# JamesKane/DecodingUsTools

Measured on NVIDIA B200. Metric: aligned Gbases/s CallableLoci pileup, higher is better.
Workload: dtype u8/u32 integer

## Files before the change

decodingustools_b200/csrc/callable_loci_b200.cu:

```cuda
#include "../../include/callable_loci_b200.h"
#include "clb_kernels.cuh"
#include "clb_fast.cuh"

#include <dlfcn.h>

#include <algorithm>
#include <cstdarg>
#include <cstdio>
#include <cstdlib>
#include <cstring>
#include <string>
#include <vector>

using namespace clb;

namespace {

struct DevBuf {
    void *p = nullptr;
    size_t cap = 0;
};

struct EvPair { cudaEvent_t a, b; };

// ... 13 lines not shown

    bool in_contig = false, finished = false;
    int32_t tid = 0;
    std::string name;
    uint32_t contig_len = 0, largest = 0, region_start = 0, region_end = 0;
    uint32_t n_windows = 0, windows_done = 0;
    uint32_t stride = 0, n_bins = 0;
    uint32_t dh_next = 0, dh_n = 0;
    uint32_t dh_fetched = 0;
    bool long_mode = false, span_on_device = false;
    uint64_t n_reads = 0, n_cigar = 0, n_qual = 0;
    long long last_pos = -1;

    DevBuf pos, flag, mapq, cigar_off, cigar, qual_off, qual, read_end, cigar_ckpt;
    DevBuf nmask, ref_ascii;
    DevBuf stats_padded, counters, rec, win_tab, win_rec, win_out, deep_list, intervals, misc;
    DevBuf gen_list, blk_tot, dhist;
    DevBuf dbg_raw, dbg_qc, dbg_low, dbg_state, timing;
    uint32_t rec_cap = 0;
    bool dbg = false;

    clb_interval *h_intervals = nullptr;
    size_t h_intervals_cap = 0;
    std::vector<unsigned long long> h_counters;
    std::vector<uint32_t> h_bins;
    uint32_t *h_misc = nullptr;
    uint64_t h2d_bytes = 0, d2h_bytes = 0;
    uint32_t launches = 0;
    uint64_t n_intervals = 0;
};

enum { M_CURSOR = 0, M_ERR = 1, M_NTOTAL = 2, M_DEEP = 3, M_GEN_COUNT = 4, M_GEN_TAKEN = 5, M_RESET_WORDS = 6, M_MAXSPAN = 7, M_MAXQLEN = 8, M_WORDS = 9 };

namespace {

int fail(clb_ctx *c, int code, const char *fmt, ...) {
    char buf[512];
    va_list ap; va_start(ap, fmt); vsnprintf(buf, sizeof buf, fmt, ap); va_end(ap);
    if (c) c->err = buf;
    return code;
}

#define CU(call)                                                                                              \
    do {                                                                                                      \
        cudaError_t e_ = (call);                                                                              \
        if (e_ != cudaSuccess) return fail(ctx, CLB_E_CUDA, "%s failed: %s (%s:%d)", #call, cudaGetErrorString(e_), __FILE__, __LINE__); \
    } while (0)
// ... 33 lines not shown
KParams make_params(clb_ctx *c) {
    KParams P{};
    P.pos = (const int32_t *)c->pos.p; P.flag = (const uint16_t *)c->flag.p; P.mapq = (const uint8_t *)c->mapq.p;
    P.cigar_off = (const uint32_t *)c->cigar_off.p; P.cigar = (const uint32_t *)c->cigar.p;
    P.qual_off = (const uint64_t *)c->qual_off.p; P.qual = (const uint8_t *)c->qual.p; P.qual_bytes = c->qual.cap;
    P.read_end = c->long_mode ? (const uint32_t *)c->read_end.p : nullptr;
    P.cigar_ckpt = c->long_mode ? (const uint2 *)c->cigar_ckpt.p : nullptr;
    P.nmask = (const uint32_t *)c->nmask.p;
    P.region_start = c->region_start; P.region_end = c->region_end;
    P.min_depth = c->opt.min_depth; P.max_depth = c->opt.max_depth; P.min_depth_for_low_mapq = c->opt.min_depth_for_low_mapq;
    P.min_mapq = c->opt.min_mapping_quality; P.min_bq = c->opt.min_base_quality; P.max_low_mapq = c->opt.max_low_mapq;
    P.first_tab = c->d_first_tab;
    P.win_tables = c->d_first_tab + 65536;
    P.first_tab8 = (const uint8_t *)(c->d_first_tab + 65536) + WIN_TABLE_BYTES;
    P.win_rec = (const uint4 *)c->win_rec.p;
    P.stats = (unsigned long long *)c->stats_padded.p;
    P.bins = (unsigned long long *)c->counters.p + N_STATS;
    P.n_bins = c->n_bins; P.stride = c->stride;
    P.rec = (unsigned long long *)c->rec.p; P.rec_cap = c->rec_cap;
    P.rec_cursor = (uint32_t *)c->misc.p + M_CURSOR;
    P.win_tab = (uint2 *)c->win_tab.p;
    P.err = (uint32_t *)c->misc.p + M_ERR;
    P.deep_count = (uint32_t *)c->misc.p + M_DEEP; P.deep_list = (uint32_t *)c->deep_list.p;
    P.gen_list = (uint32_t *)c->gen_list.p;
    P.gen_count = (uint32_t *)c->misc.p + M_GEN_COUNT; P.gen_taken = (uint32_t *)c->misc.p + M_GEN_TAKEN;
    P.max_span = (const uint32_t *)c->misc.p + M_MAXSPAN;
    P.max_low_mapq_fraction = c->opt.max_low_mapq_fraction;
    P.timing = (long long *)c->timing.p;
    P.dhist = c->dh_n ? (unsigned long long *)c->dhist.p : nullptr; P.dh_n = c->dh_n;
    if (c->dbg) {
        P.dbg_raw = (uint32_t *)c->dbg_raw.p; P.dbg_qc = (uint32_t *)c->dbg_qc.p;
        P.dbg_low = (uint32_t *)c->dbg_low.p; P.dbg_state = (uint8_t *)c->dbg_state.p;
    }
    return P;
}

template <typename F>
void with_variant(bool bq_hi, bool dbg, bool hist, F &&f) {
    using T = std::true_type; using N = std::false_type;
    auto h = [&](auto b, auto d) { if (hist) f(b, d, T{}); else f(b, d, N{}); };
    if (bq_hi) { if (dbg) h(T{}, T{}); else h(T{}, N{}); }
    else { if (dbg) h(N{}, T{}); else h(N{}, N{}); }
}

int launch_windows(clb_ctx *ctx, uint32_t w0, uint32_t w1, EvPair *time_pileup = nullptr, EvPair *time_fast = nullptr) {
    if (w1 <= w0) return CLB_OK;
    const uint32_t n = w1 - w0;
    const bool all_general = ctx->force_general || ctx->long_mode;
    k_window_ranges<<<(unsigned)(((uint64_t)n * WR_LANES + 255) / 256), 256, 0, ctx->s_compute>>>(
        (const int32_t *)ctx->pos.p, (uint32_t)ctx->n_reads, ctx->region_start, ctx->region_end,
        (const uint32_t *)ctx->misc.p + M_MAXSPAN, w0, n, (const uint64_t *)ctx->qual_off.p, (const uint32_t *)ctx->cigar_off.p, ctx->stride,
        (uint4 *)ctx->win_rec.p, all_general ? 1u : 0u, (uint32_t *)ctx->gen_list.p, (uint32_t *)ctx->misc.p + M_GEN_COUNT,
        (const uint32_t *)ctx->misc.p + M_MAXQLEN);
    KParams P = make_params(ctx);
    P.win_first = w0;
    if (time_pileup) CU(cudaEventRecord(time_pileup->a, ctx->s_compute));
    const bool hi = ctx->opt.min_base_quality >= 128;
    if (!all_general) {
        if (time_fast) CU(cudaEventRecord(time_fast->a, ctx->s_compute));
        with_variant(hi, ctx->dbg, ctx->dh_n != 0, [&](auto h, auto d, auto x) {
            k_pileup_fast<decltype(h)::value, decltype(d)::value, decltype(x)::value><<<n, NT, F_SMEM, ctx->s_compute>>>(P);
        });
        if (time_fast) CU(cudaEventRecord(time_fast->b, ctx->s_compute));
        ctx->launches += 1;
    }
    const uint32_t g = (uint32_t)std::min<uint64_t>((uint64_t)ctx->n_sm * std::max(1, ctx->max_ctas_per_sm), all_general ? n : 0xffffffffu);
    with_variant(hi, ctx->dbg, ctx->dh_n != 0, [&](auto h, auto d, auto x) {
        k_pileup_general<decltype(h)::value, decltype(d)::value, decltype(x)::value><<<g, NT, SMEM_BYTES, ctx->s_compute>>>(P);
    });
    if (time_pileup) CU(cudaEventRecord(time_pileup->b, ctx->s_compute));
    ctx->launches += 2;
    CU(cudaGetLastError());
    return CLB_OK;
}

int reset_accumulators(clb_ctx *ctx) {
    CU(cudaMemsetAsync(ctx->stats_padded.p, 0, (size_t)N_STATS * STAT_STRIDE * 8, ctx->s_compute));
    CU(cudaMemsetAsync(ctx->counters.p, 0, n_counters(ctx) * 8, ctx->s_compute));
    if (ctx->dh_n) CU(cudaMemsetAsync(ctx->dhist.p, 0, (size_t)DH_SLOTS * 2 * ctx->dh_n * 8, ctx->s_compute));
    CU(cudaMemsetAsync((uint32_t *)ctx->misc.p + M_CURSOR, 0, M_RESET_WORDS * sizeof(uint32_t), ctx->s_compute));
    return CLB_OK;
}

int launch_compaction(clb_ctx *ctx) {
    if (ctx->n_windows == 0) return CLB_OK;
    {
        const KParams P = make_params(ctx);
        with_variant(ctx->opt.min_base_quality >= 128, ctx->dbg, ctx->dh_n != 0, [&](auto h, auto d, auto x) {
            k_pileup_classify_deep<decltype(h)::value, decltype(d)::value, decltype(x)::value><<<ctx->n_sm, NT, SMEM_BYTES_DEEP, ctx->s_compute>>>(P);
        });
        ctx->launches += 1;
    }
    const uint32_t n_blk = (ctx->n_windows + 1023) / 1024;
    k_scan_windows_local<<<n_blk, 1024, 0, ctx->s_compute>>>((const uint2 *)ctx->win_tab.p, ctx->n_windows, (uint32_t *)ctx->win_out.p,
                                                            (uint32_t *)ctx->blk_tot.p, (const uint32_t *)ctx->misc.p + M_ERR);
    k_scan_blocks<<<1, 1024, 0, ctx->s_compute>>>((uint32_t *)ctx->blk_tot.p, n_blk, (uint32_t *)ctx->misc.p + M_NTOTAL);
    const uint32_t warps_per_block = 8;
    k_gather_intervals<<<(ctx->n_windows + warps_per_block - 1) / warps_per_block, warps_per_block * 32, 0, ctx->s_compute>>>(
        (const unsigned long long *)ctx->rec.p, (const uint2 *)ctx->win_tab.p, (const uint32_t *)ctx->win_out.p,
        (const uint32_t *)ctx->blk_tot.p, ctx->n_windows, (IntervalOut *)ctx->intervals.p, (const uint32_t *)ctx->misc.p + M_ERR);
    k_fill_ends<<<std::max(1, ctx->n_sm * 4), 256, 0, ctx->s_compute>>>((IntervalOut *)ctx->intervals.p,
                                                                       (const uint32_t *)ctx->misc.p + M_NTOTAL, ctx->region_end,
                                                                       (const uint32_t *)ctx->misc.p + M_ERR);
    k_pack_stats<<<1, 32, 0, ctx->s_compute>>>((const unsigned long long *)ctx->stats_padded.p, (unsigned long long *)ctx->counters.p);
    ctx->launches += 5;
    if (ctx->dh_n) {
        const uint32_t n2 = 2 * ctx->dh_n;
        k_fold_depth_hist<<<(n2 + 255) / 256, 256, 0, ctx->s_compute>>>((const unsigned long long *)ctx->dhist.p, n2,
                                                                     (unsigned long long *)ctx->counters.p + N_STATS + 3 * (size_t)ctx->n_bins);
        ctx->launches += 1;
    }
    CU(cudaGetLastError());
    return CLB_OK;
}

int alloc_outputs(clb_ctx *ctx) {
    int rc;
    const size_t nw = std::max<size_t>(ctx->n_windows, 1);
    if ((rc = ensure(ctx, ctx->win_tab, nw * sizeof(uint2), false, ctx->s_compute))) return rc;
    if ((rc = ensure(ctx, ctx->win_rec, nw * 3 * sizeof(uint4), false, ctx->s_compute))) return rc;
    if ((rc = ensure(ctx, ctx->win_out, nw * 4, false, ctx->s_compute))) return rc;
    if ((rc = ensure(ctx, ctx->deep_list, nw * 4, false, ctx->s_compute))) return rc;
    if ((rc = ensure(ctx, ctx->gen_list, nw * 4, false, ctx->s_compute))) return rc;
    if ((rc = ensure(ctx, ctx->blk_tot, ((nw + 1023) / 1024 + 1) * 4, false, ctx->s_compute))) return rc;
    if ((rc = ensure(ctx, ctx->rec, (size_t)ctx->rec_cap * 8, false, ctx->s_compute))) return rc;
    if ((rc = ensure(ctx, ctx->intervals, (size_t)ctx->rec_cap * sizeof(IntervalOut), false, ctx->s_compute))) return rc;
    return CLB_OK;
}

int fetch_result(clb_ctx *ctx, clb_contig_result *out) {
    const size_t n_cnt = n_counters(ctx);
    ctx->dh_fetched = 0;
    ctx->h_counters.resize(n_cnt);
    CU(cudaMemcpyAsync(ctx->h_misc, ctx->misc.p, M_WORDS * 4, cudaMemcpyDeviceToHost, ctx->s_compute));
    CU(cudaMemcpyAsync(ctx->h_counters.data(), ctx->counters.p, n_cnt * 8, cudaMemcpyDeviceToHost, ctx->s_compute));
    CU(cudaStreamSynchronize(ctx->s_compute));
    const uint32_t e = ctx->h_misc[M_ERR];
    if (e & ERR_UNSORTED) return fail(ctx, CLB_E_INPUT, "read columns are not coordinate sorted (or pos < 0)");
    if (e & ERR_OFFSETS) return fail(ctx, CLB_E_INPUT, "cigar_off / qual_off are not monotone");
    if (e & ERR_QUAL_SPAN) return fail(ctx, CLB_E_UNSUPPORTED, "a window's candidate reads span more than 4 GiB of qualities");
    if (e & ERR_REC_OVERFLOW) return 1;
// ... 116 lines not shown
    cudaDeviceGetAttribute(&ctx->n_sm, cudaDevAttrMultiProcessorCount, device);
    if ((e = cudaMalloc((void **)&ctx->d_first_tab, 65536 * 4 + WIN_TABLE_BYTES + 256)) != cudaSuccess) { clb_destroy(ctx); return bail("cudaMalloc", e); }
    k_first_table<<<65536 / 256, 256, 0, ctx->s_compute>>>(ctx->d_first_tab, (uint8_t *)(ctx->d_first_tab + 65536) + WIN_TABLE_BYTES, opt->max_low_mapq_fraction);
    k_window_tables<<<1, 256, 0, ctx->s_compute>>>(ctx->d_first_tab + 65536, opt->max_low_mapq_fraction);
    if ((e = cudaHostAlloc((void **)&ctx->h_misc, M_WORDS * 4, cudaHostAllocDefault)) != cudaSuccess) { clb_destroy(ctx); return bail("cudaHostAlloc", e); }
    if ((e = cudaStreamSynchronize(ctx->s_compute)) != cudaSuccess) { clb_destroy(ctx); return bail("first-table kernel", e); }
    return ctx;
}

void clb_destroy(clb_ctx *ctx) {
    if (!ctx) return;
    cudaSetDevice(ctx->device);
    cudaDeviceSynchronize();
    for (DevBuf *b : {&ctx->pos, &ctx->flag, &ctx->mapq, &ctx->cigar_off, &ctx->cigar, &ctx->qual_off, &ctx->qual, &ctx->read_end, &ctx->cigar_ckpt,
                      &ctx->nmask, &ctx->ref_ascii, &ctx->stats_padded, &ctx->counters, &ctx->rec, &ctx->win_tab, &ctx->win_rec,
                      &ctx->win_out, &ctx->deep_list, &ctx->intervals, &ctx->misc, &ctx->gen_list, &ctx->blk_tot, &ctx->dhist, &ctx->dbg_raw, &ctx->dbg_qc, &ctx->dbg_low, &ctx->dbg_state, &ctx->timing})
        release(*b);
    if (ctx->d_first_tab) cudaFree(ctx->d_first_tab);
    if (ctx->h_intervals) cudaFreeHost(ctx->h_intervals);
    if (ctx->h_misc) cudaFreeHost(ctx->h_misc);
    for (auto &ep : ctx->ev_pool) { cudaEventDestroy(ep.a); cudaEventDestroy(ep.b); }
    for (auto &ep : ctx->ev_kernel) { cudaEventDestroy(ep.a); cudaEventDestroy(ep.b); }
    for (auto &ep : ctx->ev_h2d) { cudaEventDestroy(ep.a); cudaEventDestroy(ep.b); }
    for (auto &ep : ctx->ev_upload) { cudaEventDestroy(ep.a); cudaEventDestroy(ep.b); }
    if (ctx->ev_copy) cudaEventDestroy(ctx->ev_copy);
    if (ctx->s_own) cudaStreamDestroy(ctx->s_own);
    if (ctx->s_copy) cudaStreamDestroy(ctx->s_copy);
    delete ctx;
}

const char *clb_last_error(const clb_ctx *ctx) { return ctx ? ctx->err.c_str() : "null context"; }
// ... 344 lines not shown
```

decodingustools_b200/csrc/clb_fast.cuh:

```cuda
#pragma once
#include "clb_kernels.cuh"

namespace clb {

constexpr int F_CW = 520;
constexpr int F_WSTAGE = CLB_F_WSTAGE;
constexpr int F_XCAP = 96;
constexpr int F_MAXOPS = 64;
constexpr int F_LOOKBACK = 254;
constexpr int F_NFIRST = 256;
#ifndef CLB_F_MINB
#define CLB_F_MINB 4
#endif

constexpr int F_OFF_A = 0;
constexpr int F_OFF_C = F_OFF_A + WN * 4;
constexpr int F_OFF_STAGE = F_OFF_C + 4 * F_CW * 4;
constexpr int F_OFF_X = F_OFF_STAGE + NWARPS * F_WSTAGE;
constexpr int F_OFF_MASK = F_OFF_X + F_XCAP * 8;
constexpr int F_OFF_FIRST = F_OFF_MASK + 2 * 17 * 16;
constexpr int F_OFF_CTL = F_OFF_FIRST + F_NFIRST;
constexpr int F_OFF_BAR = F_OFF_CTL + 16 * 4;
constexpr size_t F_SMEM = F_OFF_BAR + NWARPS * 8;
constexpr int F_OFF_SCAN = F_OFF_STAGE;
// ... 101 lines not shown
    M.op0 = M.c1 > M.c0 ? P.cigar[M.c0] : 0xfu;
    M.op1 = M.c1 > M.c0 + 1u ? P.cigar[M.c0 + 1u] : 0xfu;
    M.op2 = M.c1 > M.c0 + 2u ? P.cigar[M.c0 + 2u] : 0xfu;
}
__device__ __forceinline__ void fmeta_load(const KParams &P, FMeta &M, uint32_t ic, uint64_t wqx) {
    M.fl = P.flag[ic]; M.c0 = P.cigar_off[ic]; M.c1 = P.cigar_off[ic + 1];
    M.ps = P.pos[ic]; M.mq = P.mapq[ic];
    M.q0 = (uint32_t)(P.qual_off[ic] - wqx); M.q1 = (uint32_t)(P.qual_off[ic + 1] - wqx);
    M.pback = P.pos[ic >= (uint32_t)F_LOOKBACK ? ic - (uint32_t)F_LOOKBACK : 0u];
}

template <bool BQ_HI, bool DBG, bool HIST = false>
__global__ void __launch_bounds__(NT, CLB_F_MINB) k_pileup_fast(const KParams P) {
    extern __shared__ __align__(16) uint8_t smem_raw[];
    const uint32_t w = P.win_first + blockIdx.x;
    const uint4 wg = P.win_rec[3 * (size_t)w + 2];
    const uint4 wr = P.win_rec[3 * (size_t)w];
    const ulonglong2 wq = *reinterpret_cast<const ulonglong2 *>(P.win_rec + 3 * (size_t)w + 1);
    const uint32_t G = wg.x;
    if (G == 0) return;
    if (*P.err & ERR_INPUT_REFUSED) return;
    CLB_STAMP(0);

    uint32_t *sA = reinterpret_cast<uint32_t *>(smem_raw + F_OFF_A);
    uint32_t *sC = reinterpret_cast<uint32_t *>(smem_raw + F_OFF_C);
    uint2 *sX = reinterpret_cast<uint2 *>(smem_raw + F_OFF_X);
    const uint4 *sMaskLo = reinterpret_cast<const uint4 *>(smem_raw + F_OFF_MASK);
    const uint4 *sMaskHi = sMaskLo + 17;
    const uint8_t *sFirst = smem_raw + F_OFF_FIRST;
    uint32_t *sScan = reinterpret_cast<uint32_t *>(smem_raw + F_OFF_SCAN);
    uint8_t *sLast = smem_raw + F_OFF_LAST;
    unsigned long long *sWStats = reinterpret_cast<unsigned long long *>(smem_raw + F_OFF_WSTATS);
    volatile uint32_t *sCtl = reinterpret_cast<volatile uint32_t *>(smem_raw + F_OFF_CTL);
    const int tid = threadIdx.x, lane = tid & 31, warp = tid >> 5;
    const uint32_t sA_s = smem_addr(sA), sC_s = smem_addr(sC);
    const uint32_t stage_s = smem_addr(smem_raw + F_OFF_STAGE) + (uint32_t)warp * F_WSTAGE;
    const uint32_t bar = smem_addr(smem_raw + F_OFF_BAR) + 8u * (uint32_t)warp;
    const uint32_t xcnt_s = smem_addr(const_cast<uint32_t *>(&sCtl[FC_XCNT]));

    const uint32_t wb0 = P.region_start + w * (uint32_t)WREAL;
    const uint32_t n_ent = min((uint32_t)WREAL, P.region_end - wb0);
    const uint32_t r_lo = wr.x, r_hi = wr.y;
    const uint32_t n_sub = wg.y;
    const uint32_t ebase = tid * PPT;

    FMeta M;
    uint32_t j = (uint32_t)warp;
    if (j < n_sub) fmeta_load(P, M, min(r_lo + j * G + (uint32_t)lane, r_hi - 1u), wq.x);
    uint32_t nm0, nm1;
    {
        const uint32_t p0 = wb0 + ebase;
        nm0 = P.nmask[p0 >> 5]; nm1 = P.nmask[(p0 >> 5) + 1];
    }
    const uint32_t max_span = r_hi > r_lo ? *P.max_span : 0u;
    if (tid == 0 && wg.w > wg.z) l2_prefetch(P.cigar, 4ull * wg.z, 4ull * wg.w, 64u << 10);
    {
        uint4 *z = reinterpret_cast<uint4 *>(smem_raw);
        for (int i = tid; i < (F_OFF_STAGE / 16); i += NT) z[i] = make_uint4(0, 0, 0, 0);
        const uint4 *msrc = reinterpret_cast<const uint4 *>(P.win_tables);
        uint4 *mdst = reinterpret_cast<uint4 *>(smem_raw + F_OFF_MASK);
        if (tid < 34) mdst[tid] = msrc[tid];
        const uint4 *fsrc = reinterpret_cast<const uint4 *>(P.first_tab8);
        uint4 *fdst = reinterpret_cast<uint4 *>(smem_raw + F_OFF_FIRST);
        if (tid >= 64 && tid < 64 + F_NFIRST / 16) fdst[tid - 64] = fsrc[tid - 64];
        if (tid < 4) sCtl[tid] = 0;
        if (lane == 0) mbar_init(bar, 1);
    }
    __syncthreads();
    CLB_STAMP(1);
    if (j < n_sub) fmeta_ops(P, M);

    const uint32_t t_low = (P.min_bq & 0x7fu) * 0x01010101u;
    const uint32_t min_mapq = P.min_mapq, max_low_mapq = P.max_low_mapq;
    uint32_t acc128 = 0;
    uint32_t acc_sum = 0, acc_mapq = 0;
    uint32_t parity = 0;

    for (; j < n_sub; j += NWARPS) {
        const uint32_t rb = r_lo + j * G, n = min(G, r_hi - rb);
        __syncwarp();
        const uint32_t q_first = __shfl_sync(FULL, M.q0, 0), q_last = __shfl_sync(FULL, M.q1, (int)n - 1);
        const uint32_t sb = q_first & ~15u;
        const uint32_t bytes = (q_last - sb + 15u) & ~15u;
// ... 139 lines not shown
```

decodingustools_b200/csrc/clb_kernels.cuh:

```cuda
#pragma once
#include <cuda_runtime.h>
#include <stdint.h>
#include <type_traits>

namespace clb {

#ifndef CLB_NT
#define CLB_NT 256
#endif
constexpr int NT = CLB_NT;
constexpr int NWARPS = NT / 32;
static_assert(NWARPS <= 32, "cross-warp prefixes are taken with one warp-wide reduction");
#ifndef CLB_PPT
#define CLB_PPT 8
#endif
#ifndef CLB_MINB
#define CLB_MINB 5
#endif
constexpr int PPT = CLB_PPT;
constexpr int WN = NT * PPT;
constexpr int WREAL = WN - 1;
constexpr int MAXSEG = 2;
constexpr int FAST_OPS = 6;
constexpr int NFIRST = 128;
// ... 21 lines not shown
    const uint32_t *cigar;
    const uint64_t *qual_off;
    const uint8_t  *qual;
    uint64_t qual_bytes;
    const uint32_t *read_end;
    const uint2    *cigar_ckpt;
    const uint32_t *nmask;
    uint32_t region_start, region_end;
    uint32_t min_depth, max_depth, min_depth_for_low_mapq;
    uint32_t min_mapq, min_bq, max_low_mapq;
    const uint32_t *first_tab;
    const uint8_t *first_tab8;
    const uint32_t *win_tables;
    double max_low_mapq_fraction;
    const uint4 *win_rec;
    uint32_t win_first;
    unsigned long long *stats;
    unsigned long long *bins;
    uint32_t n_bins, stride;
    unsigned long long *rec;
    uint32_t rec_cap;
    uint32_t *rec_cursor;
    uint2 *win_tab;
    uint32_t *err;
    uint32_t *deep_count, *deep_list;
    uint32_t *gen_list, *gen_count, *gen_taken;
    const uint32_t *max_span;
    uint32_t *dbg_raw, *dbg_qc, *dbg_low;
    uint8_t *dbg_state;
    long long *timing;
// ... 297 lines not shown
constexpr int BPR = DCAP / 64;
constexpr int CPLX_CAP = BPR * 32;
constexpr size_t SMEM_BYTES = SMEM_COUNTER_WORDS * 4 + 2 * 17 * 16 + NFIRST * 4 + NRCP * 4 + (size_t)(NWARPS * 32 + DCAP) * 8 + 64 * 4 + NT
                            + (size_t)NWARPS * N_STATS * 8 + 128 + 2 * CPLX_CAP * 4;
static_assert((size_t)KLQ * LQ_SLAB >= (size_t)WN + 32, "the u32-per-position fallback must fit in the packed low-BQ region");
constexpr size_t SMEM_BYTES_DEEP = SMEM_BYTES + (size_t)WN * 4;
constexpr size_t WIN_TABLE_BYTES = 2 * 17 * 16 + NFIRST * 4 + NRCP * 4;
static_assert(WIN_TABLE_BYTES % 16 == 0, "window tables are copied with 16-byte loads");
static_assert(SMEM_COUNTER_WORDS % 4 == 0 && LQ_SLAB % 4 == 0, "counter region is zeroed with 16-byte stores");

struct IntervalOut { uint32_t start, end; uint8_t state, soft; uint16_t pad; };

__device__ __forceinline__ unsigned long long pack_rec(uint32_t pos, uint32_t state, uint32_t soft) {
    return (unsigned long long)pos | ((unsigned long long)state << 32) | ((unsigned long long)soft << 40);
}
__device__ __forceinline__ IntervalOut unpack_rec(unsigned long long r) {
    IntervalOut iv; iv.start = (uint32_t)r; iv.end = 0; iv.state = (uint8_t)(r >> 32); iv.soft = (uint8_t)((r >> 40) & 1u); iv.pad = 0;
    return iv;
}

__device__ __forceinline__ uint32_t pack_win_y(uint32_t count, uint32_t first_state, uint32_t wsoft, uint32_t last_state) {
    return count | (first_state << 12) | (wsoft << 16) | (last_state << 20);
}
__device__ __forceinline__ uint32_t win_count(uint32_t y) { return y & 0xfffu; }
__device__ __forceinline__ uint32_t win_drop_first(const uint2 *win_tab, uint32_t w) {
    const uint32_t y = win_tab[w].y;
    if (!((y >> 16) & 1u) || w == 0) return 0u;
    return ((y >> 12) & 15u) == ((win_tab[w - 1].y >> 20) & 15u) ? 1u : 0u;
}

using stp_t = typename std::conditional<(PPT > 8), unsigned long long, uint32_t>::type;

template <typename Sum>
struct Entries {
// ... 556 lines not shown
__device__ __forceinline__ uint32_t lower_bound_pos_group(const int32_t *pos, uint32_t n, long long key, uint32_t gmask, int gl, int gbase) {
    constexpr uint32_t GS = WR_LANES;
    uint32_t lo = 0, hi = n;
    while (hi - lo > GS) {
        const uint32_t idx = lo + (uint32_t)(((unsigned long long)(hi - lo) * (unsigned)(gl + 1)) / (GS + 1u));
        const uint32_t below = (__ballot_sync(gmask, (long long)pos[idx] < key) >> gbase) & (GS == 32u ? 0xffffffffu : ((1u << GS) - 1u));
        const int c = __popc(below);
        const uint32_t lo_n = __shfl_sync(gmask, idx, gbase + max(c - 1, 0)) + 1u;
        const uint32_t hi_n = __shfl_sync(gmask, idx, gbase + min(c, (int)GS - 1));
        lo = c ? lo_n : lo; hi = c < (int)GS ? hi_n : hi;
    }
    const uint32_t i = lo + (uint32_t)gl;
    return lo + (uint32_t)__popc(__ballot_sync(gmask, i < hi && (long long)pos[i] < key) & gmask);
}

__global__ void k_window_ranges(const int32_t *pos, uint32_t n_reads, uint32_t region_start, uint32_t region_end,
                                const uint32_t *max_span_ptr, uint32_t w_first, uint32_t n_w,
                                const uint64_t *qual_off, const uint32_t *cigar_off, uint32_t stride, uint4 *win_rec,
                                uint32_t force_general, uint32_t *gen_list, uint32_t *gen_count, const uint32_t *max_qlen_ptr) {
    constexpr uint32_t GS = WR_LANES;
    const uint32_t gi = (blockIdx.x * blockDim.x + threadIdx.x) / GS;
    const int lane = threadIdx.x & 31, gl = lane & (int)(GS - 1u), gbase = lane - gl;
    const uint32_t gmask = (GS == 32u ? 0xffffffffu : ((1u << GS) - 1u)) << gbase;
    const bool real = gi < n_w;
    const uint32_t i = real ? gi : n_w - 1u;
    const uint32_t max_span = *max_span_ptr;
    const uint32_t w = w_first + i;
    const long long wb = (long long)region_start + (long long)w * WREAL - 1;
    const long long wend = min(wb + WN, (long long)region_end);
    const uint32_t r_lo = lower_bound_pos_group(pos, n_reads, wb - (long long)max_span + 1, gmask, gl, gbase);
    const uint32_t r_hi = lower_bound_pos_group(pos, n_reads, wend, gmask, gl, gbase);
    const uint32_t first_bin = stride ? (uint32_t)(wb + 1) / stride : 0u;
    const uint64_t q_lo = qual_off[r_lo] & ~15ull, q_hi = qual_off[r_hi];
    const uint32_t n_cand = r_hi - r_lo;
    bool general = force_general != 0 || (w == 0 && region_start != 0) || n_cand > 16384u || q_hi - q_lo > 0xfffffff0ull;
    const uint32_t c_lo = cigar_off[r_lo], c_hi = cigar_off[r_hi];
    if (!general && n_cand) general = (c_hi - c_lo) > 8u * n_cand + 64u;
    if (!general) {
        bool deep = false;
        for (uint32_t i2 = r_lo + 254u * (uint32_t)(gl + 1); i2 < r_hi; i2 += 254u * GS)
            deep |= (long long)pos[i2 - 254u] + (long long)max_span > (long long)pos[i2];
        general = (__ballot_sync(gmask, deep) & gmask) != 0u;
    }
    uint32_t G = 32;
    if (!general && n_cand) {
        const uint64_t total = q_hi - q_lo;
        if (total * 32u > (uint64_t)(CLB_F_WSTAGE - 16) * n_cand) G = (uint32_t)(((uint64_t)(CLB_F_WSTAGE - 16) * n_cand) / total);
        const uint32_t max_qlen = *max_qlen_ptr;
        bool ok = G >= 4u && max_qlen != 0u && (uint64_t)G * max_qlen + 32u <= (uint64_t)CLB_F_WSTAGE;
        for (int tries = 0; tries < 4 && G >= 4u && !ok; tries++) {
            uint32_t worst = 0;
            for (uint32_t b = r_lo + (uint32_t)gl * G; b < r_hi; b += GS * G) {
                const uint64_t bytes = (qual_off[min(b + G, r_hi)] - (qual_off[b] & ~15ull) + 15ull) & ~15ull;
                worst = max(worst, (uint32_t)min(bytes, (uint64_t)0xffffffffu));
            }
            ok = __reduce_max_sync(gmask, worst) <= (uint32_t)CLB_F_WSTAGE;
            if (!ok) G -= max(1u, G / 8u);
        }
        if (!ok) general = true;
    }
    if (real && gl == 0) {
        win_rec[3 * (size_t)w] = make_uint4(r_lo, r_hi, first_bin, stride ? (uint32_t)((long long)(first_bin + 1) * stride - wb) : 0xffffffffu);
        *reinterpret_cast<ulonglong2 *>(win_rec + 3 * (size_t)w + 1) = make_ulonglong2(q_lo, q_hi);
        win_rec[3 * (size_t)w + 2] = make_uint4(general ? 0u : G, general ? 0u : (n_cand + G - 1u) / G, c_lo, c_hi);
        if (general) gen_list[atomicAdd(gen_count, 1u)] = w;
    }
}

__global__ void k_read_end(const int32_t *pos, const uint32_t *cigar_off, const uint32_t *cigar, uint32_t r0, uint32_t r1,
                           uint32_t *read_end, uint32_t *max_span) {
    const uint32_t r = r0 + blockIdx.x * blockDim.x + threadIdx.x;
    uint32_t span = 0;
    if (r < r1) {
        for (uint32_t c = cigar_off[r]; c < cigar_off[r + 1]; c++) { const uint32_t v = cigar[c]; if (op_ref(v & 15u)) span += v >> 4; }
        if (read_end) read_end[r] = (uint32_t)pos[r] + span;
    }
    span = __reduce_max_sync(FULL, span);
    if (max_span && (threadIdx.x & 31) == 0 && span) atomicMax(max_span, span);
}

// ... 78 lines not shown
            out[4 * t + q] = ml; out[17 * 4 + 4 * t + q] = mh;
        }
    }
    for (uint32_t i = t; i < (uint32_t)NFIRST; i += blockDim.x) out[2 * 17 * 4 + i] = first_low(i, fraction);
    for (uint32_t i = t; i < (uint32_t)NRCP; i += blockDim.x) out[2 * 17 * 4 + NFIRST + i] = i > 1 ? 0xffffffffu / i + 1u : 0u;
}

__global__ void k_first_table(uint32_t *first_tab, uint8_t *first_tab8, double fraction) {
    const uint32_t raw = blockIdx.x * blockDim.x + threadIdx.x;
    if (raw >= 65536u) return;
    const uint32_t f = first_low(raw, fraction);
    first_tab[raw] = f;
    if (raw < 256u) first_tab8[raw] = (uint8_t)min(f, 255u);
}

__global__ void __launch_bounds__(1024) k_scan_windows_local(const uint2 *win_tab, uint32_t n_w, uint32_t *win_out, uint32_t *blk_tot,
                                                             const uint32_t *err) {
    __shared__ uint32_t sW[32];
    const int tid = threadIdx.x, lane = tid & 31, warp = tid >> 5;
    if (*err & ERR_RESULT_INVALID) return;
    const uint32_t i = blockIdx.x * 1024u + tid;
    const uint32_t v = i < n_w ? win_count(win_tab[i].y) - win_drop_first(win_tab, i) : 0u;
    uint32_t inc = v;
#pragma unroll
    for (int dd = 1; dd < 32; dd <<= 1) { const uint32_t t = __shfl_up_sync(FULL, inc, dd); if (lane >= dd) inc += t; }
    if (lane == 31) sW[warp] = inc;
    __syncthreads();
    const uint32_t wt = sW[lane];
    const uint32_t off = __reduce_add_sync(FULL, lane < warp ? wt : 0u);
    if (i < n_w) win_out[i] = off + inc - v;
    if (tid == 1023) blk_tot[blockIdx.x] = off + inc;
}
__global__ void __launch_bounds__(1024) k_scan_blocks(uint32_t *blk_tot, uint32_t n_blk, uint32_t *n_total) {
    __shared__ uint32_t sW[32];
    __shared__ uint32_t sCarry;
    const int tid = threadIdx.x, lane = tid & 31, warp = tid >> 5;
    if (tid == 0) sCarry = 0;
    __syncthreads();
    for (uint32_t base = 0; base < n_blk; base += 1024u) {
        const uint32_t i = base + tid;
        const uint32_t v = i < n_blk ? blk_tot[i] : 0u;
        uint32_t inc = v;
#pragma unroll
        for (int dd = 1; dd < 32; dd <<= 1) { const uint32_t t = __shfl_up_sync(FULL, inc, dd); if (lane >= dd) inc += t; }
        if (lane == 31) sW[warp] = inc;
        __syncthreads();
        const uint32_t wt = sW[lane];
        const uint32_t off = sCarry + __reduce_add_sync(FULL, lane < warp ? wt : 0u);
        if (i < n_blk) blk_tot[i] = off + inc - v;
        __syncthreads();
        if (tid == 1023) sCarry = off + inc;
        __syncthreads();
    }
    if (tid == 0) *n_total = sCarry;
}

__global__ void k_gather_intervals(const unsigned long long *rec, const uint2 *win_tab, const uint32_t *win_out, const uint32_t *blk_off,
                                   uint32_t n_w, IntervalOut *out, const uint32_t *err) {
    const uint32_t w = (blockIdx.x * blockDim.x + threadIdx.x) >> 5;
    const int lane = threadIdx.x & 31;
    if (w >= n_w || (*err & (ERR_REC_OVERFLOW | ERR_RESULT_INVALID))) return;
    const uint2 t = win_tab[w];
    const uint32_t skip = win_drop_first(win_tab, w);
    const uint32_t o = blk_off[w >> 10] + win_out[w], cnt = win_count(t.y) - skip;
    for (uint32_t i = lane; i < cnt; i += 32) {
        out[o + i] = unpack_rec(rec[t.x + skip + i]);
    }
}

__global__ void k_fill_ends(IntervalOut *out, const uint32_t *n_total, uint32_t region_end, const uint32_t *err) {
    if (*err & (ERR_REC_OVERFLOW | ERR_RESULT_INVALID)) return;
    const uint32_t n = *n_total;
    for (uint32_t i = blockIdx.x * blockDim.x + threadIdx.x; i < n; i += gridDim.x * blockDim.x)
        out[i].end = (i + 1 < n) ? out[i + 1].start : region_end;
}

__global__ void k_pack_stats(const unsigned long long *stats_padded, unsigned long long *counters) {
    if (threadIdx.x < N_STATS) counters[threadIdx.x] = stats_padded[threadIdx.x * STAT_STRIDE];
}

__global__ void k_fold_depth_hist(const unsigned long long *slots, uint32_t n2, unsigned long long *out) {
    for (uint32_t i = blockIdx.x * blockDim.x + threadIdx.x; i < n2; i += gridDim.x * blockDim.x) {
        unsigned long long t = 0;
#pragma unroll
        for (int k = 0; k < DH_SLOTS; k++) t += slots[(size_t)k * n2 + i];
        out[i] = t;
    }
}

}
```

Measured before the change: 2698.

## Overlap window ranging with pileup via PDL and fuse compaction into single-pass scan

```diff
diff --git a/decodingustools_b200/csrc/callable_loci_b200.cu b/decodingustools_b200/csrc/callable_loci_b200.cu
--- a/decodingustools_b200/csrc/callable_loci_b200.cu
+++ b/decodingustools_b200/csrc/callable_loci_b200.cu
@@ -51,10 +51,11 @@
 
     DevBuf pos, flag, mapq, cigar_off, cigar, qual_off, qual, read_end, cigar_ckpt;
     DevBuf nmask, ref_ascii;
-    DevBuf stats_padded, counters, rec, win_tab, win_rec, win_out, deep_list, intervals, misc;
-    DevBuf gen_list, blk_tot, dhist;
+    DevBuf stats_padded, counters, rec, win_tab, win_rec, win_ready, deep_list, intervals, misc;
+    DevBuf gen_list, tile_st, dhist;
     DevBuf dbg_raw, dbg_qc, dbg_low, dbg_state, timing;
     uint32_t rec_cap = 0;
+    uint32_t epoch = 0;
     bool dbg = false;
 
     clb_interval *h_intervals = nullptr;
@@ -67,7 +68,7 @@
     uint64_t n_intervals = 0;
 };
 
-enum { M_CURSOR = 0, M_ERR = 1, M_NTOTAL = 2, M_DEEP = 3, M_GEN_COUNT = 4, M_GEN_TAKEN = 5, M_RESET_WORDS = 6, M_MAXSPAN = 7, M_MAXQLEN = 8, M_WORDS = 9 };
+enum { M_CURSOR = 0, M_ERR = 1, M_NTOTAL = 2, M_DEEP = 3, M_GEN_COUNT = 4, M_GEN_TAKEN = 5, M_TILES = 6, M_RESET_WORDS = 7, M_MAXSPAN = 8, M_MAXQLEN = 9, M_WORDS = 10 };
 
 namespace {
 
@@ -131,6 +132,7 @@
     P.win_tables = c->d_first_tab + 65536;
     P.first_tab8 = (const uint8_t *)(c->d_first_tab + 65536) + WIN_TABLE_BYTES;
     P.win_rec = (const uint4 *)c->win_rec.p;
+    P.win_ready = (const uint32_t *)c->win_ready.p;
     P.stats = (unsigned long long *)c->stats_padded.p;
     P.bins = (unsigned long long *)c->counters.p + N_STATS;
     P.n_bins = c->n_bins; P.stride = c->stride;
@@ -160,24 +162,38 @@
     else { if (dbg) h(N{}, T{}); else h(N{}, N{}); }
 }
 
+uint32_t next_epoch(clb_ctx *ctx) { ctx->epoch = ctx->epoch % 0x3fffffffu + 1u; return ctx->epoch; }
+
 int launch_windows(clb_ctx *ctx, uint32_t w0, uint32_t w1, EvPair *time_pileup = nullptr, EvPair *time_fast = nullptr) {
     if (w1 <= w0) return CLB_OK;
     const uint32_t n = w1 - w0;
     const bool all_general = ctx->force_general || ctx->long_mode;
-    k_window_ranges<<<(unsigned)(((uint64_t)n * WR_LANES + 255) / 256), 256, 0, ctx->s_compute>>>(
+    const uint32_t epoch = next_epoch(ctx);
+    const uint64_t full = ((uint64_t)n * WR_LANES + WR_THREADS - 1) / WR_THREADS;
+    const unsigned wr_grid = (unsigned)(all_general ? full : std::min<uint64_t>(full, (uint64_t)std::max(1, ctx->n_sm)));
+    if (time_pileup) CU(cudaEventRecord(time_pileup->a, ctx->s_compute));
+    if (time_fast && !all_general) CU(cudaEventRecord(time_fast->a, ctx->s_compute));
+    k_window_ranges<<<wr_grid, WR_THREADS, 0, ctx->s_compute>>>(
         (const int32_t *)ctx->pos.p, (uint32_t)ctx->n_reads, ctx->region_start, ctx->region_end,
         (const uint32_t *)ctx->misc.p + M_MAXSPAN, w0, n, (const uint64_t *)ctx->qual_off.p, (const uint32_t *)ctx->cigar_off.p, ctx->stride,
-        (uint4 *)ctx->win_rec.p, all_general ? 1u : 0u, (uint32_t *)ctx->gen_list.p, (uint32_t *)ctx->misc.p + M_GEN_COUNT,
-        (const uint32_t *)ctx->misc.p + M_MAXQLEN);
+        (uint4 *)ctx->win_rec.p, (uint32_t *)ctx->win_ready.p, epoch, all_general ? 1u : 0u, (uint32_t *)ctx->gen_list.p,
+        (uint32_t *)ctx->misc.p + M_GEN_COUNT, (const uint32_t *)ctx->misc.p + M_MAXQLEN);
     KParams P = make_params(ctx);
     P.win_first = w0;
-    if (time_pileup) CU(cudaEventRecord(time_pileup->a, ctx->s_compute));
+    P.epoch = epoch;
     const bool hi = ctx->opt.min_base_quality >= 128;
     if (!all_general) {
-        if (time_fast) CU(cudaEventRecord(time_fast->a, ctx->s_compute));
+        cudaLaunchAttribute attr[1];
+        attr[0].id = cudaLaunchAttributeProgrammaticStreamSerialization;
+        attr[0].val.programmaticStreamSerializationAllowed = 1;
+        cudaLaunchConfig_t cfg = {};
+        cfg.gridDim = dim3(n); cfg.blockDim = dim3(NT); cfg.dynamicSmemBytes = F_SMEM; cfg.stream = ctx->s_compute;
+        cfg.attrs = attr; cfg.numAttrs = 1;
+        cudaError_t e = cudaSuccess;
         with_variant(hi, ctx->dbg, ctx->dh_n != 0, [&](auto h, auto d, auto x) {
-            k_pileup_fast<decltype(h)::value, decltype(d)::value, decltype(x)::value><<<n, NT, F_SMEM, ctx->s_compute>>>(P);
+            e = cudaLaunchKernelEx(&cfg, k_pileup_fast<decltype(h)::value, decltype(d)::value, decltype(x)::value>, P);
         });
+        CU(e);
         if (time_fast) CU(cudaEventRecord(time_fast->b, ctx->s_compute));
         ctx->launches += 1;
     }
@@ -208,19 +224,13 @@
         });
         ctx->launches += 1;
     }
-    const uint32_t n_blk = (ctx->n_windows + 1023) / 1024;
-    k_scan_windows_local<<<n_blk, 1024, 0, ctx->s_compute>>>((const uint2 *)ctx->win_tab.p, ctx->n_windows, (uint32_t *)ctx->win_out.p,
-                                                            (uint32_t *)ctx->blk_tot.p, (const uint32_t *)ctx->misc.p + M_ERR);
-    k_scan_blocks<<<1, 1024, 0, ctx->s_compute>>>((uint32_t *)ctx->blk_tot.p, n_blk, (uint32_t *)ctx->misc.p + M_NTOTAL);
-    const uint32_t warps_per_block = 8;
-    k_gather_intervals<<<(ctx->n_windows + warps_per_block - 1) / warps_per_block, warps_per_block * 32, 0, ctx->s_compute>>>(
-        (const unsigned long long *)ctx->rec.p, (const uint2 *)ctx->win_tab.p, (const uint32_t *)ctx->win_out.p,
-        (const uint32_t *)ctx->blk_tot.p, ctx->n_windows, (IntervalOut *)ctx->intervals.p, (const uint32_t *)ctx->misc.p + M_ERR);
-    k_fill_ends<<<std::max(1, ctx->n_sm * 4), 256, 0, ctx->s_compute>>>((IntervalOut *)ctx->intervals.p,
-                                                                       (const uint32_t *)ctx->misc.p + M_NTOTAL, ctx->region_end,
-                                                                       (const uint32_t *)ctx->misc.p + M_ERR);
-    k_pack_stats<<<1, 32, 0, ctx->s_compute>>>((const unsigned long long *)ctx->stats_padded.p, (unsigned long long *)ctx->counters.p);
-    ctx->launches += 5;
+    const uint32_t n_tiles = (ctx->n_windows + CT_WIN - 1) / CT_WIN;
+    k_compact_intervals<<<n_tiles, CT_WIN, 0, ctx->s_compute>>>(
+        (const unsigned long long *)ctx->rec.p, (const uint2 *)ctx->win_tab.p, ctx->n_windows, (IntervalOut *)ctx->intervals.p,
+        (unsigned long long *)ctx->tile_st.p, next_epoch(ctx), (uint32_t *)ctx->misc.p + M_TILES, (uint32_t *)ctx->misc.p + M_NTOTAL,
+        ctx->region_end, (const uint32_t *)ctx->misc.p + M_ERR, (const unsigned long long *)ctx->stats_padded.p,
+        (unsigned long long *)ctx->counters.p);
+    ctx->launches += 1;
     if (ctx->dh_n) {
         const uint32_t n2 = 2 * ctx->dh_n;
         k_fold_depth_hist<<<(n2 + 255) / 256, 256, 0, ctx->s_compute>>>((const unsigned long long *)ctx->dhist.p, n2,
@@ -236,12 +246,14 @@
     const size_t nw = std::max<size_t>(ctx->n_windows, 1);
     if ((rc = ensure(ctx, ctx->win_tab, nw * sizeof(uint2), false, ctx->s_compute))) return rc;
     if ((rc = ensure(ctx, ctx->win_rec, nw * 3 * sizeof(uint4), false, ctx->s_compute))) return rc;
-    if ((rc = ensure(ctx, ctx->win_out, nw * 4, false, ctx->s_compute))) return rc;
+    if ((rc = ensure(ctx, ctx->win_ready, nw * 4, false, ctx->s_compute))) return rc;
     if ((rc = ensure(ctx, ctx->deep_list, nw * 4, false, ctx->s_compute))) return rc;
     if ((rc = ensure(ctx, ctx->gen_list, nw * 4, false, ctx->s_compute))) return rc;
-    if ((rc = ensure(ctx, ctx->blk_tot, ((nw + 1023) / 1024 + 1) * 4, false, ctx->s_compute))) return rc;
+    if ((rc = ensure(ctx, ctx->tile_st, (nw + CT_WIN - 1) / CT_WIN * 8, false, ctx->s_compute))) return rc;
     if ((rc = ensure(ctx, ctx->rec, (size_t)ctx->rec_cap * 8, false, ctx->s_compute))) return rc;
     if ((rc = ensure(ctx, ctx->intervals, (size_t)ctx->rec_cap * sizeof(IntervalOut), false, ctx->s_compute))) return rc;
+    CU(cudaMemsetAsync(ctx->win_ready.p, 0, nw * 4, ctx->s_compute));
+    CU(cudaMemsetAsync(ctx->tile_st.p, 0, (nw + CT_WIN - 1) / CT_WIN * 8, ctx->s_compute));
     return CLB_OK;
 }
 
@@ -388,7 +400,7 @@
     cudaDeviceSynchronize();
     for (DevBuf *b : {&ctx->pos, &ctx->flag, &ctx->mapq, &ctx->cigar_off, &ctx->cigar, &ctx->qual_off, &ctx->qual, &ctx->read_end, &ctx->cigar_ckpt,
                       &ctx->nmask, &ctx->ref_ascii, &ctx->stats_padded, &ctx->counters, &ctx->rec, &ctx->win_tab, &ctx->win_rec,
-                      &ctx->win_out, &ctx->deep_list, &ctx->intervals, &ctx->misc, &ctx->gen_list, &ctx->blk_tot, &ctx->dhist, &ctx->dbg_raw, &ctx->dbg_qc, &ctx->dbg_low, &ctx->dbg_state, &ctx->timing})
+                      &ctx->win_ready, &ctx->deep_list, &ctx->intervals, &ctx->misc, &ctx->gen_list, &ctx->tile_st, &ctx->dhist, &ctx->dbg_raw, &ctx->dbg_qc, &ctx->dbg_low, &ctx->dbg_state, &ctx->timing})
         release(*b);
     if (ctx->d_first_tab) cudaFree(ctx->d_first_tab);
     if (ctx->h_intervals) cudaFreeHost(ctx->h_intervals);
diff --git a/decodingustools_b200/csrc/clb_fast.cuh b/decodingustools_b200/csrc/clb_fast.cuh
--- a/decodingustools_b200/csrc/clb_fast.cuh
+++ b/decodingustools_b200/csrc/clb_fast.cuh
@@ -139,13 +139,6 @@
 __global__ void __launch_bounds__(NT, CLB_F_MINB) k_pileup_fast(const KParams P) {
     extern __shared__ __align__(16) uint8_t smem_raw[];
     const uint32_t w = P.win_first + blockIdx.x;
-    const uint4 wg = P.win_rec[3 * (size_t)w + 2];
-    const uint4 wr = P.win_rec[3 * (size_t)w];
-    const ulonglong2 wq = *reinterpret_cast<const ulonglong2 *>(P.win_rec + 3 * (size_t)w + 1);
-    const uint32_t G = wg.x;
-    if (G == 0) return;
-    if (*P.err & ERR_INPUT_REFUSED) return;
-    CLB_STAMP(0);
 
     uint32_t *sA = reinterpret_cast<uint32_t *>(smem_raw + F_OFF_A);
     uint32_t *sC = reinterpret_cast<uint32_t *>(smem_raw + F_OFF_C);
@@ -165,20 +158,12 @@
 
     const uint32_t wb0 = P.region_start + w * (uint32_t)WREAL;
     const uint32_t n_ent = min((uint32_t)WREAL, P.region_end - wb0);
-    const uint32_t r_lo = wr.x, r_hi = wr.y;
-    const uint32_t n_sub = wg.y;
     const uint32_t ebase = tid * PPT;
-
-    FMeta M;
-    uint32_t j = (uint32_t)warp;
-    if (j < n_sub) fmeta_load(P, M, min(r_lo + j * G + (uint32_t)lane, r_hi - 1u), wq.x);
     uint32_t nm0, nm1;
     {
         const uint32_t p0 = wb0 + ebase;
         nm0 = P.nmask[p0 >> 5]; nm1 = P.nmask[(p0 >> 5) + 1];
     }
-    const uint32_t max_span = r_hi > r_lo ? *P.max_span : 0u;
-    if (tid == 0 && wg.w > wg.z) l2_prefetch(P.cigar, 4ull * wg.z, 4ull * wg.w, 64u << 10);
     {
         uint4 *z = reinterpret_cast<uint4 *>(smem_raw);
         for (int i = tid; i < (F_OFF_STAGE / 16); i += NT) z[i] = make_uint4(0, 0, 0, 0);
@@ -191,7 +176,24 @@
         if (tid < 4) sCtl[tid] = 0;
         if (lane == 0) mbar_init(bar, 1);
     }
+    wait_window_ready(P.win_ready + w, P.epoch);
     __syncthreads();
+    CLB_STAMP(0);
+    const uint4 wg = P.win_rec[3 * (size_t)w + 2];
+    const uint4 wr = P.win_rec[3 * (size_t)w];
+    const ulonglong2 wq = *reinterpret_cast<const ulonglong2 *>(P.win_rec + 3 * (size_t)w + 1);
+    const uint32_t G = wg.x;
+    if (G == 0) return;
+    if (*P.err & ERR_INPUT_REFUSED) return;
+
+    const uint32_t r_lo = wr.x, r_hi = wr.y;
+    const uint32_t n_sub = wg.y;
+
+    FMeta M;
+    uint32_t j = (uint32_t)warp;
+    if (j < n_sub) fmeta_load(P, M, min(r_lo + j * G + (uint32_t)lane, r_hi - 1u), wq.x);
+    const uint32_t max_span = r_hi > r_lo ? *P.max_span : 0u;
+    if (tid == 0 && wg.w > wg.z) l2_prefetch(P.cigar, 4ull * wg.z, 4ull * wg.w, 64u << 10);
     CLB_STAMP(1);
     if (j < n_sub) fmeta_ops(P, M);
 
diff --git a/decodingustools_b200/csrc/clb_kernels.cuh b/decodingustools_b200/csrc/clb_kernels.cuh
--- a/decodingustools_b200/csrc/clb_kernels.cuh
+++ b/decodingustools_b200/csrc/clb_kernels.cuh
@@ -59,6 +59,8 @@
     const uint32_t *win_tables;
     double max_low_mapq_fraction;
     const uint4 *win_rec;
+    const uint32_t *win_ready;
+    uint32_t epoch;
     uint32_t win_first;
     unsigned long long *stats;
     unsigned long long *bins;
@@ -386,10 +388,7 @@
 __device__ __forceinline__ unsigned long long pack_rec(uint32_t pos, uint32_t state, uint32_t soft) {
     return (unsigned long long)pos | ((unsigned long long)state << 32) | ((unsigned long long)soft << 40);
 }
-__device__ __forceinline__ IntervalOut unpack_rec(unsigned long long r) {
-    IntervalOut iv; iv.start = (uint32_t)r; iv.end = 0; iv.state = (uint8_t)(r >> 32); iv.soft = (uint8_t)((r >> 40) & 1u); iv.pad = 0;
-    return iv;
-}
+__device__ __forceinline__ uint32_t rec_state_word(unsigned long long r) { return (uint32_t)(r >> 32) & 0x1ffu; }
 
 __device__ __forceinline__ uint32_t pack_win_y(uint32_t count, uint32_t first_state, uint32_t wsoft, uint32_t last_state) {
     return count | (first_state << 12) | (wsoft << 16) | (last_state << 20);
@@ -976,56 +975,73 @@
     return lo + (uint32_t)__popc(__ballot_sync(gmask, i < hi && (long long)pos[i] < key) & gmask);
 }
 
-__global__ void k_window_ranges(const int32_t *pos, uint32_t n_reads, uint32_t region_start, uint32_t region_end,
-                                const uint32_t *max_span_ptr, uint32_t w_first, uint32_t n_w,
-                                const uint64_t *qual_off, const uint32_t *cigar_off, uint32_t stride, uint4 *win_rec,
-                                uint32_t force_general, uint32_t *gen_list, uint32_t *gen_count, const uint32_t *max_qlen_ptr) {
+constexpr int WR_THREADS = 192;
+__global__ void __launch_bounds__(WR_THREADS, 8) k_window_ranges(const int32_t *pos, uint32_t n_reads, uint32_t region_start, uint32_t region_end,
+                                                       const uint32_t *max_span_ptr, uint32_t w_first, uint32_t n_w,
+                                                       const uint64_t *qual_off, const uint32_t *cigar_off, uint32_t stride, uint4 *win_rec,
+                                                       uint32_t *win_ready, uint32_t epoch,
+                                                       uint32_t force_general, uint32_t *gen_list, uint32_t *gen_count, const uint32_t *max_qlen_ptr) {
+    asm volatile("griddepcontrol.launch_dependents;" ::: "memory");
     constexpr uint32_t GS = WR_LANES;
-    const uint32_t gi = (blockIdx.x * blockDim.x + threadIdx.x) / GS;
     const int lane = threadIdx.x & 31, gl = lane & (int)(GS - 1u), gbase = lane - gl;
     const uint32_t gmask = (GS == 32u ? 0xffffffffu : ((1u << GS) - 1u)) << gbase;
-    const bool real = gi < n_w;
-    const uint32_t i = real ? gi : n_w - 1u;
     const uint32_t max_span = *max_span_ptr;
-    const uint32_t w = w_first + i;
-    const long long wb = (long long)region_start + (long long)w * WREAL - 1;
-    const long long wend = min(wb + WN, (long long)region_end);
-    const uint32_t r_lo = lower_bound_pos_group(pos, n_reads, wb - (long long)max_span + 1, gmask, gl, gbase);
-    const uint32_t r_hi = lower_bound_pos_group(pos, n_reads, wend, gmask, gl, gbase);
-    const uint32_t first_bin = stride ? (uint32_t)(wb + 1) / stride : 0u;
-    const uint64_t q_lo = qual_off[r_lo] & ~15ull, q_hi = qual_off[r_hi];
-    const uint32_t n_cand = r_hi - r_lo;
-    bool general = force_general != 0 || (w == 0 && region_start != 0) || n_cand > 16384u || q_hi - q_lo > 0xfffffff0ull;
-    const uint32_t c_lo = cigar_off[r_lo], c_hi = cigar_off[r_hi];
-    if (!general && n_cand) general = (c_hi - c_lo) > 8u * n_cand + 64u;
-    if (!general) {
-        bool deep = false;
-        for (uint32_t i2 = r_lo + 254u * (uint32_t)(gl + 1); i2 < r_hi; i2 += 254u * GS)
-            deep |= (long long)pos[i2 - 254u] + (long long)max_span > (long long)pos[i2];
-        general = (__ballot_sync(gmask, deep) & gmask) != 0u;
-    }
-    uint32_t G = 32;
-    if (!general && n_cand) {
-        const uint64_t total = q_hi - q_lo;
-        if (total * 32u > (uint64_t)(CLB_F_WSTAGE - 16) * n_cand) G = (uint32_t)(((uint64_t)(CLB_F_WSTAGE - 16) * n_cand) / total);
-        const uint32_t max_qlen = *max_qlen_ptr;
-        bool ok = G >= 4u && max_qlen != 0u && (uint64_t)G * max_qlen + 32u <= (uint64_t)CLB_F_WSTAGE;
-        for (int tries = 0; tries < 4 && G >= 4u && !ok; tries++) {
-            uint32_t worst = 0;
-            for (uint32_t b = r_lo + (uint32_t)gl * G; b < r_hi; b += GS * G) {
-                const uint64_t bytes = (qual_off[min(b + G, r_hi)] - (qual_off[b] & ~15ull) + 15ull) & ~15ull;
-                worst = max(worst, (uint32_t)min(bytes, (uint64_t)0xffffffffu));
-            }
-            ok = __reduce_max_sync(gmask, worst) <= (uint32_t)CLB_F_WSTAGE;
-            if (!ok) G -= max(1u, G / 8u);
-        }
-        if (!ok) general = true;
-    }
-    if (real && gl == 0) {
-        win_rec[3 * (size_t)w] = make_uint4(r_lo, r_hi, first_bin, stride ? (uint32_t)((long long)(first_bin + 1) * stride - wb) : 0xffffffffu);
-        *reinterpret_cast<ulonglong2 *>(win_rec + 3 * (size_t)w + 1) = make_ulonglong2(q_lo, q_hi);
-        win_rec[3 * (size_t)w + 2] = make_uint4(general ? 0u : G, general ? 0u : (n_cand + G - 1u) / G, c_lo, c_hi);
-        if (general) gen_list[atomicAdd(gen_count, 1u)] = w;
+    const uint32_t max_qlen = *max_qlen_ptr;
+    const uint32_t n_groups = gridDim.x * blockDim.x / GS;
+    const uint32_t warp_first = (blockIdx.x * blockDim.x + (threadIdx.x & ~31u)) / GS;
+    for (uint32_t g0 = warp_first; g0 < n_w; g0 += n_groups) {
+        const uint32_t gi = g0 + (uint32_t)(gbase / (int)GS);
+        const bool real = gi < n_w;
+        const uint32_t i = real ? gi : n_w - 1u;
+        const uint32_t w = w_first + i;
+        const long long wb = (long long)region_start + (long long)w * WREAL - 1;
+        const long long wend = min(wb + WN, (long long)region_end);
+        const uint32_t r_lo = lower_bound_pos_group(pos, n_reads, wb - (long long)max_span + 1, gmask, gl, gbase);
+        const uint32_t r_hi = lower_bound_pos_group(pos, n_reads, wend, gmask, gl, gbase);
+        const uint32_t first_bin = stride ? (uint32_t)(wb + 1) / stride : 0u;
+        const uint64_t q_lo = qual_off[r_lo] & ~15ull, q_hi = qual_off[r_hi];
+        const uint32_t n_cand = r_hi - r_lo;
+        bool general = force_general != 0 || (w == 0 && region_start != 0) || n_cand > 16384u || q_hi - q_lo > 0xfffffff0ull;
+        const uint32_t c_lo = cigar_off[r_lo], c_hi = cigar_off[r_hi];
+        if (!general && n_cand) general = (c_hi - c_lo) > 8u * n_cand + 64u;
+        if (!general) {
+            bool deep = false;
+            for (uint32_t i2 = r_lo + 254u * (uint32_t)(gl + 1); i2 < r_hi; i2 += 254u * GS)
+                deep |= (long long)pos[i2 - 254u] + (long long)max_span > (long long)pos[i2];
+            general = (__ballot_sync(gmask, deep) & gmask) != 0u;
+        }
+        uint32_t G = 32;
+        if (!general && n_cand) {
+            const uint64_t total = q_hi - q_lo;
+            if (total * 32u > (uint64_t)(CLB_F_WSTAGE - 16) * n_cand) G = (uint32_t)(((uint64_t)(CLB_F_WSTAGE - 16) * n_cand) / total);
+            bool ok = G >= 4u && max_qlen != 0u && (uint64_t)G * max_qlen + 32u <= (uint64_t)CLB_F_WSTAGE;
+            for (int tries = 0; tries < 4 && G >= 4u && !ok; tries++) {
+                uint32_t worst = 0;
+                for (uint32_t b = r_lo + (uint32_t)gl * G; b < r_hi; b += GS * G) {
+                    const uint64_t bytes = (qual_off[min(b + G, r_hi)] - (qual_off[b] & ~15ull) + 15ull) & ~15ull;
+                    worst = max(worst, (uint32_t)min(bytes, (uint64_t)0xffffffffu));
+                }
+                ok = __reduce_max_sync(gmask, worst) <= (uint32_t)CLB_F_WSTAGE;
+                if (!ok) G -= max(1u, G / 8u);
+            }
+            if (!ok) general = true;
+        }
+        if (real && gl == 0) {
+            win_rec[3 * (size_t)w] = make_uint4(r_lo, r_hi, first_bin, stride ? (uint32_t)((long long)(first_bin + 1) * stride - wb) : 0xffffffffu);
+            *reinterpret_cast<ulonglong2 *>(win_rec + 3 * (size_t)w + 1) = make_ulonglong2(q_lo, q_hi);
+            win_rec[3 * (size_t)w + 2] = make_uint4(general ? 0u : G, general ? 0u : (n_cand + G - 1u) / G, c_lo, c_hi);
+            if (general) gen_list[atomicAdd(gen_count, 1u)] = w;
+            asm volatile("st.release.gpu.global.u32 [%0], %1;" :: "l"(win_ready + w), "r"(epoch) : "memory");
+        }
+    }
+}
+
+__device__ __forceinline__ void wait_window_ready(const uint32_t *ready, uint32_t epoch) {
+    uint32_t v;
+    asm volatile("ld.acquire.gpu.global.u32 %0, [%1];" : "=r"(v) : "l"(ready) : "memory");
+    while (v != epoch) {
+        __nanosleep(128);
+        asm volatile("ld.acquire.gpu.global.u32 %0, [%1];" : "=r"(v) : "l"(ready) : "memory");
     }
 }
 
@@ -1134,69 +1150,81 @@
     if (raw < 256u) first_tab8[raw] = (uint8_t)min(f, 255u);
 }
 
-__global__ void __launch_bounds__(1024) k_scan_windows_local(const uint2 *win_tab, uint32_t n_w, uint32_t *win_out, uint32_t *blk_tot,
-                                                             const uint32_t *err) {
-    __shared__ uint32_t sW[32];
+constexpr int CT_WIN = 256;
+__device__ __forceinline__ unsigned long long tile_word(uint32_t epoch, uint32_t flag, uint32_t v) {
+    return (unsigned long long)v | ((unsigned long long)(flag | (epoch << 2)) << 32);
+}
+
+__global__ void __launch_bounds__(CT_WIN) k_compact_intervals(const unsigned long long *rec, const uint2 *win_tab, uint32_t n_w,
+                                                               IntervalOut *out, unsigned long long *tile_st, uint32_t epoch,
+                                                               uint32_t *ticket, uint32_t *n_total, uint32_t region_end, const uint32_t *err,
+                                                               const unsigned long long *stats_padded, unsigned long long *counters) {
+    __shared__ uint32_t sIncl[CT_WIN], sSrc[CT_WIN], sW[CT_WIN / 32];
+    __shared__ uint32_t sTile, sBase;
     const int tid = threadIdx.x, lane = tid & 31, warp = tid >> 5;
-    if (*err & ERR_RESULT_INVALID) return;
-    const uint32_t i = blockIdx.x * 1024u + tid;
-    const uint32_t v = i < n_w ? win_count(win_tab[i].y) - win_drop_first(win_tab, i) : 0u;
+    if (blockIdx.x == 0 && tid < N_STATS) counters[tid] = stats_padded[tid * STAT_STRIDE];
+    if (*err & (ERR_REC_OVERFLOW | ERR_RESULT_INVALID)) return;
+    if (tid == 0) sTile = atomicAdd(ticket, 1u);
+    __syncthreads();
+    const uint32_t tile = sTile, n_tiles = (n_w + CT_WIN - 1) / CT_WIN;
+    const uint32_t w = tile * CT_WIN + (uint32_t)tid;
+    uint32_t v = 0, src = 0;
+    if (w < n_w) {
+        const uint2 t = win_tab[w];
+        const uint32_t skip = win_drop_first(win_tab, w);
+        v = win_count(t.y) - skip; src = t.x + skip;
+    }
     uint32_t inc = v;
 #pragma unroll
-    for (int dd = 1; dd < 32; dd <<= 1) { const uint32_t t = __shfl_up_sync(FULL, inc, dd); if (lane >= dd) inc += t; }
+    for (int dd = 1; dd < 32; dd <<= 1) { const uint32_t t1 = __shfl_up_sync(FULL, inc, dd); if (lane >= dd) inc += t1; }
     if (lane == 31) sW[warp] = inc;
     __syncthreads();
-    const uint32_t wt = sW[lane];
-    const uint32_t off = __reduce_add_sync(FULL, lane < warp ? wt : 0u);
-    if (i < n_w) win_out[i] = off + inc - v;
-    if (tid == 1023) blk_tot[blockIdx.x] = off + inc;
-}
-__global__ void __launch_bounds__(1024) k_scan_blocks(uint32_t *blk_tot, uint32_t n_blk, uint32_t *n_total) {
-    __shared__ uint32_t sW[32];
-    __shared__ uint32_t sCarry;
-    const int tid = threadIdx.x, lane = tid & 31, warp = tid >> 5;
-    if (tid == 0) sCarry = 0;
+    inc += __reduce_add_sync(FULL, lane < warp ? sW[lane] : 0u);
+    sIncl[tid] = inc;
+    sSrc[tid] = src - (inc - v);
     __syncthreads();
-    for (uint32_t base = 0; base < n_blk; base += 1024u) {
-        const uint32_t i = base + tid;
-        const uint32_t v = i < n_blk ? blk_tot[i] : 0u;
-        uint32_t inc = v;
-#pragma unroll
-        for (int dd = 1; dd < 32; dd <<= 1) { const uint32_t t = __shfl_up_sync(FULL, inc, dd); if (lane >= dd) inc += t; }
-        if (lane == 31) sW[warp] = inc;
-        __syncthreads();
-        const uint32_t wt = sW[lane];
-        const uint32_t off = sCarry + __reduce_add_sync(FULL, lane < warp ? wt : 0u);
-        if (i < n_blk) blk_tot[i] = off + inc - v;
-        __syncthreads();
-        if (tid == 1023) sCarry = off + inc;
-        __syncthreads();
-    }
-    if (tid == 0) *n_total = sCarry;
-}
-
-__global__ void k_gather_intervals(const unsigned long long *rec, const uint2 *win_tab, const uint32_t *win_out, const uint32_t *blk_off,
-                                   uint32_t n_w, IntervalOut *out, const uint32_t *err) {
-    const uint32_t w = (blockIdx.x * blockDim.x + threadIdx.x) >> 5;
-    const int lane = threadIdx.x & 31;
-    if (w >= n_w || (*err & (ERR_REC_OVERFLOW | ERR_RESULT_INVALID))) return;
-    const uint2 t = win_tab[w];
-    const uint32_t skip = win_drop_first(win_tab, w);
-    const uint32_t o = blk_off[w >> 10] + win_out[w], cnt = win_count(t.y) - skip;
-    for (uint32_t i = lane; i < cnt; i += 32) {
-        out[o + i] = unpack_rec(rec[t.x + skip + i]);
-    }
-}
-
-__global__ void k_fill_ends(IntervalOut *out, const uint32_t *n_total, uint32_t region_end, const uint32_t *err) {
-    if (*err & (ERR_REC_OVERFLOW | ERR_RESULT_INVALID)) return;
-    const uint32_t n = *n_total;
-    for (uint32_t i = blockIdx.x * blockDim.x + threadIdx.x; i < n; i += gridDim.x * blockDim.x)
-        out[i].end = (i + 1 < n) ? out[i + 1].start : region_end;
-}
-
-__global__ void k_pack_stats(const unsigned long long *stats_padded, unsigned long long *counters) {
-    if (threadIdx.x < N_STATS) counters[threadIdx.x] = stats_padded[threadIdx.x * STAT_STRIDE];
+    const uint32_t total = sIncl[CT_WIN - 1];
+    if (warp == 0) {
+        volatile unsigned long long *st = tile_st;
+        uint32_t excl = 0;
+        if (tile == 0) {
+            if (lane == 0) st[0] = tile_word(epoch, 2u, total);
+        } else {
+            if (lane == 0) st[tile] = tile_word(epoch, 1u, total);
+            for (int p0 = (int)tile - 1;; p0 -= 32) {
+                const int p = p0 - lane;
+                unsigned long long s = tile_word(epoch, 2u, 0u);
+                if (p >= 0) {
+                    do { s = st[p]; } while ((uint32_t)(s >> 34) != (epoch & 0x3fffffffu) || ((s >> 32) & 3u) == 0u);
+                }
+                const uint32_t inclusive = __ballot_sync(FULL, ((s >> 32) & 3u) == 2u);
+                const int stop = inclusive ? __ffs(inclusive) - 1 : 31;
+                excl += __reduce_add_sync(FULL, lane <= stop ? (uint32_t)s : 0u);
+                if (inclusive) break;
+            }
+            if (lane == 0) st[tile] = tile_word(epoch, 2u, excl + total);
+        }
+        if (lane == 0) {
+            sBase = excl;
+            if (tile == n_tiles - 1u) {
+                *n_total = excl + total;
+                if (excl + total) out[excl + total - 1u].end = region_end;
+            }
+        }
+    }
+    __syncthreads();
+    const uint32_t base = sBase;
+    uint32_t *o32 = reinterpret_cast<uint32_t *>(out);
+    for (uint32_t o = (uint32_t)tid; o < total; o += CT_WIN) {
+        uint32_t k = 0;
+#pragma unroll
+        for (uint32_t step = CT_WIN / 2; step; step >>= 1) if (sIncl[k + step - 1u] <= o) k += step;
+        const unsigned long long r = rec[sSrc[k] + o];
+        const uint32_t g = base + o, start = (uint32_t)r;
+        o32[3 * (size_t)g] = start;
+        o32[3 * (size_t)g + 2] = rec_state_word(r);
+        if (g) o32[3 * (size_t)g - 2] = start;
+    }
 }
 
 __global__ void k_fold_depth_hist(const unsigned long long *slots, uint32_t n2, unsigned long long *out) {
```

Result: slower. 2386 (median of 6 runs) (-11.6%).
